# rsokolovskii/fl_scaling_sc_ldpc

Measured on AMD Instinct MI355X. Metric: MC codeword trials/sec, (4,8) SC-LDPC L=50 N=1000 eps=0.48 full BP, higher is better.
Workload: dtype u32

## Files before the change

### fl_scaling_sc_ldpc_amd/_lib.py

```python
import ctypes as C
import os

import numpy as np

HERE = os.path.dirname(os.path.abspath(__file__))
LIB_PATH = os.environ.get("SCLDPC_LIB_PATH") or os.path.join(HERE, "libscldpc_hip.so")

NCOUNTERS = 8
NRUN = 9
MAX_CAPS = 16
NPEELRUN = 8
PEELRUN_NAMES = ("trials", "fuckups", "lost", "fuckups_exp", "lost_exp", "blocks_exp")
COUNTER_NAMES = ("num_erasures", "num_blocks_err", "num_erasures_exp", "num_blocks_err_exp",
                 "num_erasures_p1", "iterations", "status", "channel_erasures")
RUN_NAMES = ("users_err", "frame_err", "frame_err_p1", "block_err", "users_err_exp", "frame_err_exp",
             "block_err_exp", "frames", "iterations")

EXPORTS = (
    "scldpc_abi_version", "scldpc_last_error", "scldpc_device_count",
    "scldpc_sample_glibc_host", "scldpc_glibc_state_bytes", "scldpc_glibc_state_init",
    "scldpc_glibc_state_reset_perm", "scldpc_sample_glibc_next_host",
    "scldpc_sample_philox_device", "scldpc_full_bp_device", "scldpc_sw_bp_device",
    "scldpc_accumulate_run_device", "scldpc_full_bp_lds_bytes",
    "scldpc_sample_philox_device_adj16", "scldpc_full_bp_device_adj16", "scldpc_sw_bp_device_adj16",
# ... 9 lines not shown
    "scldpc_sw_bp_ring_supported", "scldpc_cn_sockets_device", "scldpc_sw_bp_ring_device",
    "scldpc_accumulate_peel_device", "scldpc_clear_channel_range_device",
    "scldpc_stream_glibc_next_host", "scldpc_stream_run_device_inputs_at",
    "scldpc_full_bp_sock16_supported", "scldpc_full_bp_fixpoint_device_sock16", "scldpc_full_bp_device_sock16",
    "scldpc_full_bp_traj_device_cn16", "scldpc_full_bp_traj_device_sock16",
    "scldpc_full_bp_caps_device_cn16", "scldpc_full_bp_caps_device_sock16",
    "scldpc_full_bp_wide_supported", "scldpc_full_bp_device_wide", "scldpc_full_bp_traj_device_wide",
    "scldpc_full_bp_deg_supported", "scldpc_full_bp_deg_wide_supported", "scldpc_full_bp_fixpoint_device_deg",
    "scldpc_full_bp_device_deg", "scldpc_full_bp_traj_device_deg", "scldpc_full_bp_device_deg_wide",
    "scldpc_full_bp_traj_device_deg_wide",
    "scldpc_full_bp_caps_device_wide", "scldpc_full_bp_caps_device_deg", "scldpc_full_bp_caps_device_deg_wide",
    "scldpc_sw_bp_ring_deg_supported", "scldpc_sw_bp_ring_device_deg",
    "scldpc_stream_supported",
    "scldpc_swc_bp_ring_supported", "scldpc_swc_bp_ring_device",
    "scldpc_sample_philox_adj16_sock_supported", "scldpc_sample_philox_device_adj16_sock",
)


class ScldpcError(RuntimeError):
    pass


class CodeParams(C.Structure):
    _fields_ = [("dv", C.c_int32), ("dc", C.c_int32), ("L", C.c_int32), ("cns_pos", C.c_int32),
                ("vns_pos", C.c_int32)]

    @property
    def n(self):
        return self.vns_pos * self.L

    @property
    def nk(self):
        return (self.L + self.dv - 1) * self.cns_pos

    @property
    def nw(self):
        return (self.n + 31) // 32

    @property
    def edges(self):
        return self.n * self.dv

    def key(self):
        return (self.dv, self.dc, self.L, self.cns_pos, self.vns_pos)


_lib = None


def lib():
    global _lib
    if _lib is not None:
        return _lib
    if not os.path.exists(LIB_PATH):
        raise ScldpcError(f"{LIB_PATH} is missing — build it with `make -C fl_scaling_sc_ldpc_amd/csrc` "
                          "(hipcc, gfx950).  There is no CPU fallback.")
    import torch
    L = C.CDLL(LIB_PATH)
    P = C.POINTER
# ... 8 lines not shown
    L.scldpc_glibc_state_init.argtypes = [pp, u32, vp]
    L.scldpc_glibc_state_reset_perm.argtypes = [pp, vp]
    L.scldpc_sample_glibc_next_host.argtypes = [pp, vp, dbl, i32, vp, i32, vp, vp]
    L.scldpc_workspace_bytes.argtypes = [i32, pp, i32, i32, i32]
    L.scldpc_workspace_bytes.restype = i64
    L.scldpc_sample_philox_device.argtypes = [pp, u64, u64, i32, dbl, i32, vp, vp, vp, vp, u64, vp]
    L.scldpc_sample_philox_ensemble_device.argtypes = [pp, i32, u64, u64, i32, dbl, i32, vp, vp, vp, vp]
    L.scldpc_full_bp_fixpoint_device.argtypes = [pp, i32, vp, vp, i32, vp, vp, vp, u64, vp]
    L.scldpc_full_bp_fixpoint_device_adj16.argtypes = L.scldpc_full_bp_fixpoint_device.argtypes
    L.scldpc_sample_philox_cn16_supported.argtypes = [pp]
    L.scldpc_full_bp_cn16_supported.argtypes = [pp]
    L.scldpc_sample_philox_device_cn16.argtypes = [pp, u64, u64, i32, dbl, i32, vp, vp, vp, vp, vp]
    L.scldpc_sample_philox_sock16_supported.argtypes = [pp]
    L.scldpc_sample_philox_device_sock16.argtypes = [pp, u64, u64, i32, dbl, i32, vp, vp, vp, vp, vp]
    L.scldpc_sample_philox_adj16_sock_supported.argtypes = [pp]
    L.scldpc_sample_philox_device_adj16_sock.argtypes = [pp, u64, u64, i32, dbl, i32, vp, vp, vp, vp, vp, u64, vp]
    L.scldpc_full_bp_fixpoint_device_cn16.argtypes = [pp, i32, vp, vp, vp, i32, vp, vp, vp]
    L.scldpc_full_bp_device_cn16.argtypes = [pp, i32, vp, vp, vp, i32, i32, vp, vp, vp]
    L.scldpc_full_bp_sock16_supported.argtypes = [pp]
    L.scldpc_full_bp_fixpoint_device_sock16.argtypes = L.scldpc_full_bp_fixpoint_device_cn16.argtypes
    L.scldpc_full_bp_device_sock16.argtypes = L.scldpc_full_bp_device_cn16.argtypes
    L.scldpc_full_bp_traj_device_cn16.argtypes = [pp, i32, vp, vp, vp, i32, i32, vp, vp, i32, vp, vp]
    L.scldpc_full_bp_traj_device_sock16.argtypes = L.scldpc_full_bp_traj_device_cn16.argtypes
    L.scldpc_full_bp_caps_device_cn16.argtypes = [pp, i32, vp, vp, vp, i32, vp, i32, vp, vp]
    L.scldpc_full_bp_caps_device_sock16.argtypes = L.scldpc_full_bp_caps_device_cn16.argtypes
    L.scldpc_full_bp_wide_supported.argtypes = [pp]
    L.scldpc_full_bp_device_wide.argtypes = L.scldpc_full_bp_device_cn16.argtypes
    L.scldpc_full_bp_traj_device_wide.argtypes = L.scldpc_full_bp_traj_device_cn16.argtypes
    L.scldpc_full_bp_deg_supported.argtypes = [pp]
    L.scldpc_full_bp_deg_wide_supported.argtypes = [pp]
# ... 53 lines not shown
```

### fl_scaling_sc_ldpc_amd/csrc/sampler_v2.hip

```cpp
#include "common.h"
#include "kernel_util.h"
#include "philox.h"
#include <algorithm>
#include <cstdlib>

namespace {

using scldpc_dev::philox4x32_10;
using scldpc_dev::wave_inclusive_scan;

constexpr int kThreads = 1024;
constexpr int kWaves = kThreads / 64;
constexpr int kMaxDoped = 32;
constexpr int kWorkCap = 1024;

struct S2Args {
    int L, cns_pos, vns_pos, n, S, D, nb, nw;
    int ntrials;
    int force_exact;
    int ndoped;
    int doped[kMaxDoped];
    uint32_t seed_lo, seed_hi;
    unsigned long long trial0;
    uint32_t thresh;
    int off_gpk, off_fix, off_stage, off_wsum;
    uint16_t *vn_adj16;
    uint16_t *cn_adj16;
    uint32_t *chan;
};

template <int KMAX, int ROWS, int CNMODE, bool PERSIST = false>
__global__ __launch_bounds__(kThreads, KMAX == 1 ? 8 : 4) __attribute__((amdgpu_num_sgpr(72))) void sample_philox_v2_kernel(const S2Args a)
{
    constexpr int DV = 4, DC_SHIFT = 3, E = 4 * KMAX;
    constexpr int LG = ROWS == 1 ? 10 : ROWS == 2 ? 11 : ROWS == 4 ? 12 : 13;
    constexpr int KSHIFT = 32 - LG - 2;
    constexpr bool INCL = KMAX == 1;
    static_assert(ROWS * kThreads == (1 << LG) && (INCL ? ROWS <= 4 : ROWS == 8), "ROWS is 1, 2, 4 (KMAX 1) or 8 (KMAX 2)");
    extern __shared__ uint32_t lds[];
    uint32_t *hist = lds;
    uint32_t *gpk = lds + a.off_gpk;
    uint16_t *fix = reinterpret_cast<uint16_t *>(lds + a.off_fix);
    uint16_t *stage = reinterpret_cast<uint16_t *>(lds + a.off_stage);
    uint32_t *wsum = lds + a.off_wsum;
    uint32_t *wl = wsum + 32;

    const int tid = threadIdx.x, lane = tid & 63, wave = tid >> 6;
    const int S = a.S, nb = a.nb;
    const int ncalls = S >> 2;
    bool own[KMAX];
#pragma unroll
    for (int k = 0; k < KMAX; k++) own[k] = tid + k * kThreads < ncalls;
    auto sock = [&](int e) { return (uint32_t)((tid + (e >> 2) * kThreads) * 4 + (e & 3)); };
    auto stage_entry = [&](int p, uint32_t sck) -> uint16_t {
        const int u = (int)(sck & 3u), t = (int)(sck >> 2);
        if ((unsigned)(p - u) >= (unsigned)a.L) return (uint16_t)0xFFFFu;
        return CNMODE == 1 ? (uint16_t)((p - u) * a.vns_pos + t) : (uint16_t)sck;
    };

    auto nib_sum = [](uint32_t x) {
        const uint32_t v = (x & 0x0F0Fu) + ((x >> 4) & 0x0F0Fu);
        return (v + (v >> 8)) & 0xFFu;
    };
    auto load_words = [&](uint32_t (&x)[ROWS]) {
        if constexpr (ROWS % 4 == 0) {
#pragma unroll
            for (int r = 0; r < ROWS / 4; r++) {
                const uint4 q = reinterpret_cast<const uint4 *>(hist)[tid * (ROWS / 4) + r];
// ... 18 lines not shown
    const unsigned long long trial = a.trial0 + (unsigned long long)tr;
    const uint32_t t_lo = (uint32_t)trial, t_hi = (uint32_t)(trial >> 32);
    uint32_t rowP[KMAX], rowQ[KMAX], rowR[KMAX];
#pragma unroll
    for (int k = 0; k < KMAX; k++) rowP[k] = rowQ[k] = rowR[k] = 0;
    uint32_t nxt[E];
#pragma unroll
    for (int k = 0; k < KMAX; k++) {
        uint32_t r[4] = {0, 0, 0, 0};
        if (own[k]) philox4x32_10((uint32_t)(tid + k * kThreads), 0u, t_lo, t_hi, a.seed_lo, a.seed_hi, r);
#pragma unroll
        for (int u = 0; u < 4; u++) nxt[4 * k + u] = r[u];
    }
    for (int p = 0; p < a.D; p++) {
        STAMP(0);
        uint32_t key[E], slot[E], crowded = 0;
        auto word_of = [](uint32_t k) { return (k >> KSHIFT) & ~3u; };
        auto nib_of = [](uint32_t k) { return (k >> (KSHIFT - 2)) & 12u; };
#pragma unroll
        for (int e = 0; e < E; e++) {
            key[e] = nxt[e];
            const uint32_t sh = nib_of(key[e]);
            uint32_t *w = reinterpret_cast<uint32_t *>(reinterpret_cast<char *>(hist) + word_of(key[e]));
            slot[e] = (atomicAdd(w, (own[e >> 2] ? 1u : 0u) << sh) >> sh) & 0xFu;
            if constexpr (!INCL) crowded = max(crowded, slot[e]);
        }
        if (!INCL && crowded >= 15u) wsum[kWaves + 1] = 1u;
        __syncthreads();
        STAMP(1);

        bool ranked;
        if constexpr (INCL) {
            uint32_t x[ROWS], t20[ROWS], tot20 = 0;
            load_words(x);
#pragma unroll
            for (int r = 0; r < ROWS; r++) {
                x[r] *= 0x111110u;
                t20[r] = x[r] & 0xF00000u;
                tot20 += t20[r];
            }
            const uint32_t tot = tot20 >> 20, inc = wave_inclusive_scan(tot);
            if (lane == 63) wsum[wave] = inc;
            __syncthreads();
            uint32_t winc = lane < kWaves ? wsum[lane] : 0u;
            const uint32_t wt = winc;
            winc += (uint32_t)__builtin_amdgcn_update_dpp(0, (int)winc, 0x111, 0xF, 0xF, false);
            winc += (uint32_t)__builtin_amdgcn_update_dpp(0, (int)winc, 0x112, 0xF, 0xF, false);
            winc += (uint32_t)__builtin_amdgcn_update_dpp(0, (int)winc, 0x114, 0xF, 0xF, false);
            winc += (uint32_t)__builtin_amdgcn_update_dpp(0, (int)winc, 0x118, 0xF, 0xF, false);
            ranked = __builtin_amdgcn_readlane((int)winc, kWaves - 1) == S;
            uint32_t pre20 = (inc - tot + (uint32_t)__builtin_amdgcn_readlane((int)(winc - wt), wave)) << 20;
#pragma unroll
            for (int r = 0; r < ROWS; r++) {
                x[r] = (x[r] & 0xFFFF0u) | pre20;
                pre20 += t20[r];
            }
            store_words(x);
        } else {
            uint32_t x[ROWS], v[ROWS], tot = 0;
            load_words(x);
#pragma unroll
            for (int r = 0; r < ROWS; r++) v[r] = 0;
            if constexpr (ROWS % 2 == 0) {
#pragma unroll
                for (int r = 0; r < ROWS; r += 2) {
                    const uint32_t y = x[r] | (x[r + 1] << 16);
                    const uint32_t sb = (y & 0x0F0F0F0Fu) + ((y >> 4) & 0x0F0F0F0Fu);
                    v[r] = (sb & 0xFFu) + ((sb >> 8) & 0xFFu);
                    v[r + 1] = ((sb >> 16) & 0xFFu) + (sb >> 24);
                    tot += v[r] + v[r + 1];
// ... 6 lines not shown
            const uint32_t inc = wave_inclusive_scan(tot);
            if (lane == 63) wsum[wave] = inc;
            __syncthreads();
            const uint32_t wt = lane < kWaves ? wsum[lane] : 0u;
            const uint32_t winc = wave_inclusive_scan(wt);
            uint32_t pre = inc - tot + (uint32_t)__builtin_amdgcn_readlane((int)(winc - wt), wave);
#pragma unroll
            for (int r = 0; r < ROWS; r++) { x[r] |= pre << 16; pre += v[r]; }
            store_words(x);
        }
        __syncthreads();
        if constexpr (!INCL) ranked = wsum[kWaves + 1] == 0u;
        STAMP(2);

        if (ranked) {
            uint32_t rk[E], g0a[E], g1a[E];
            bool st[E];
            if constexpr (INCL) {
                uint32_t h[E];
#pragma unroll
                for (int e = 0; e < E; e++) h[e] = *reinterpret_cast<const uint32_t *>(reinterpret_cast<const char *>(hist) + word_of(key[e]));
#pragma unroll
                for (int e = 0; e < E; e++) {
                    const uint32_t t = h[e] >> nib_of(key[e]), pre = h[e] >> 20;
                    g0a[e] = pre + (t & 0xFu);
                    g1a[e] = pre + ((t >> 4) & 0xFu);
                    rk[e] = g0a[e] + slot[e];
                    st[e] = own[e >> 2] && ((g0a[e] ^ (g1a[e] - 1u)) >> DC_SHIFT) != 0u;
                }
            } else {
                uint32_t h[E];
#pragma unroll
                for (int e = 0; e < E; e++) h[e] = hist[own[e >> 2] ? (key[e] >> KSHIFT) >> 2 : 0u];
#pragma unroll
                for (int e = 0; e < E; e++) {
                    const uint32_t k4 = ((key[e] >> KSHIFT) & 3u) * 4u, x = h[e];
                    const uint32_t below = x & ((1u << k4) - 1u);
                    g0a[e] = (x >> 16) + (below & 0xFu) + ((below >> 4) & 0xFu) + ((below >> 8) & 0xFu);
                    g1a[e] = g0a[e] + ((x >> k4) & 0xFu);
                    rk[e] = g0a[e] + slot[e];
                    st[e] = own[e >> 2] && ((g1a[e] - 1u) >> DC_SHIFT) != (g0a[e] >> DC_SHIFT);
                }
            }
            if constexpr (INCL) {
                unsigned long long vote[E], anyv = 0;
                int total = 0;
#pragma unroll
                for (int e = 0; e < E; e++) { vote[e] = __builtin_amdgcn_ballot_w64(st[e]); anyv |= vote[e]; total += __builtin_popcountll(vote[e]); }
                if (anyv) {
                    int base = 0;
                    if (lane == 0) base = atomicAdd(reinterpret_cast<int *>(&wsum[kWaves]), total);
                    base = __builtin_amdgcn_readfirstlane(base);
                    const bool fits = base + total <= kWorkCap;
#pragma unroll
                    for (int e = 0; e < E; e++) {
                        if (st[e]) {
                            const uint32_t w = __builtin_amdgcn_mbcnt_hi((uint32_t)(vote[e] >> 32),
                                                                         __builtin_amdgcn_mbcnt_lo((uint32_t)vote[e], (uint32_t)base));
                            const uint32_t pk = (key[e] << LG) | sock(e);
                            gpk[rk[e]] = pk;
                            if (fits) { wl[2 * w] = g0a[e] | (g1a[e] << 16); wl[2 * w + 1] = pk; }
                        }
                        base += __builtin_popcountll(vote[e]);
                    }
                }
            } else {
                uint32_t smask = 0;
#pragma unroll
                for (int e = 0; e < E; e++) smask |= (st[e] ? 1u : 0u) << e;
                while (smask) {
                    const uint32_t e = (uint32_t)__ffs((int)smask) - 1u;
                    smask &= smask - 1u;
                    uint32_t ky = key[0], r0 = rk[0], g0 = g0a[0], g1 = g1a[0];
#pragma unroll
                    for (int f = 1; f < E; f++)
                        if (e == (uint32_t)f) { ky = key[f]; r0 = rk[f]; g0 = g0a[f]; g1 = g1a[f]; }
                    const uint32_t pk = (ky << LG) | (uint32_t)((tid + (int)(e >> 2) * kThreads) * 4 + (int)(e & 3u));
                    gpk[r0] = pk;
                    const int w = atomicAdd(reinterpret_cast<int *>(&wsum[kWaves]), 1);
                    if (w < kWorkCap) { wl[2 * w] = g0 | (g1 << 16); wl[2 * w + 1] = pk; }
                }
            }
#pragma unroll
            for (int k = 0; k < KMAX; k++) {
                if (!own[k]) continue;
                uint2 v;
                v.x = (rk[4 * k] >> DC_SHIFT) | ((rk[4 * k + 1] >> DC_SHIFT) << 16);
                v.y = (rk[4 * k + 2] >> DC_SHIFT) | ((rk[4 * k + 3] >> DC_SHIFT) << 16);
                reinterpret_cast<uint2 *>(fix)[tid + k * kThreads] = v;
            }
            if constexpr (CNMODE != 0) {
#pragma unroll
                for (int k = 0; k < KMAX; k++) {
                    if (!own[k]) continue;
#pragma unroll
                    for (int u = 0; u < 4; u++) stage[rk[4 * k + u]] = stage_entry(p, sock(4 * k + u));
                }
            }
        }
        __syncthreads();
        STAMP(3);

        {
            uint32_t z[ROWS];
#pragma unroll
            for (int r = 0; r < ROWS; r++) z[r] = 0;
            store_words(z);
            int nwork = (int)wsum[kWaves];
            const bool exact = !ranked || nwork > kWorkCap || a.force_exact == p || a.force_exact == -2;
            if (exact) {
                asm volatile("; ledger: cold");
                nwork = 0;
#pragma unroll
                for (int e = 0; e < E; e++) if (own[e >> 2]) gpk[sock(e)] = key[e];
                __syncthreads();
                uint32_t xr[E];
#pragma unroll
                for (int e = 0; e < E; e++) xr[e] = 0;
                for (int s2 = 0; s2 < S; s2++) {
                    const uint32_t k2 = gpk[s2];
#pragma unroll
                    for (int e = 0; e < E; e++) xr[e] += (k2 < key[e]) || (k2 == key[e] && (uint32_t)s2 < sock(e));
                }
#pragma unroll
                for (int k = 0; k < KMAX; k++) {
                    if (!own[k]) continue;
                    uint2 v;
                    v.x = (xr[4 * k] >> DC_SHIFT) | ((xr[4 * k + 1] >> DC_SHIFT) << 16);
                    v.y = (xr[4 * k + 2] >> DC_SHIFT) | ((xr[4 * k + 3] >> DC_SHIFT) << 16);
                    reinterpret_cast<uint2 *>(fix)[tid + k * kThreads] = v;
                    if constexpr (CNMODE != 0) {
#pragma unroll
                        for (int u = 0; u < 4; u++) stage[xr[4 * k + u]] = stage_entry(p, sock(4 * k + u));
                    }
                }
            }
            for (int w = tid; w < nwork; w += kThreads) {
                const uint32_t ea = wl[2 * w], pk = wl[2 * w + 1];
                uint32_t r = ea & 0xFFFFu;
#pragma unroll 1
                for (uint32_t m = ea & 0xFFFFu; m < (ea >> 16); m++) r += gpk[m] < pk;
                const uint32_t sck = pk & ((1u << LG) - 1u);
                if constexpr (CNMODE != 0) stage[r] = stage_entry(p, sck);
                fix[sck] = (uint16_t)(r >> DC_SHIFT);
            }
        }
        if (p + 1 < a.D) {
            uint32_t k_lo = a.seed_lo, k_hi = a.seed_hi;
            asm volatile("" : "+s"(k_lo), "+s"(k_hi));
#pragma unroll
            for (int k = 0; k < KMAX; k++) {
                uint32_t r[4] = {0, 0, 0, 0};
                if (own[k]) philox4x32_10((uint32_t)(tid + k * kThreads), (uint32_t)(p + 1), t_lo, t_hi, k_lo, k_hi, r);
#pragma unroll
                for (int u = 0; u < 4; u++) nxt[4 * k + u] = r[u];
            }
        }
        __syncthreads();
        if (tid == 0) { wsum[kWaves] = 0; wsum[kWaves + 1] = 0; }
        STAMP(4);

        const int qpos = p - (DV - 1);
#pragma unroll
        for (int k = 0; k < KMAX; k++) {
            uint2 c = make_uint2(0u, 0u);
            if (own[k]) c = reinterpret_cast<const uint2 *>(fix)[tid + k * kThreads];
            if (qpos >= 0 && own[k]) {
                const size_t j = (size_t)tr * a.n + (size_t)qpos * a.vns_pos + (size_t)(tid + k * kThreads);
// ... 31 lines not shown
            if (lo < hi) word &= ~(((hi - lo) == 32 ? 0xFFFFFFFFu : ((1u << (hi - lo)) - 1u)) << lo);
        }
        chan[w] = word;
    }
    STAMP(6);
    };
    if constexpr (PERSIST) {
        for (int tr = blockIdx.x; tr < a.ntrials; tr += gridDim.x) {
            sample_trial(tr);
            __syncthreads();
        }
    } else {
        sample_trial((int)blockIdx.x);
    }
    STAMP_FLUSH();
}


__device__ __forceinline__ uint32_t wl_entry_vn(const S2Args &a, int p, uint32_t sck)
{
    return (uint32_t)((p - (int)(sck & 3u)) * a.vns_pos + (int)(sck >> 2));
}

template <int LG, int CNMODE>
__global__ __launch_bounds__(kThreads, 8) __attribute__((amdgpu_num_sgpr(72))) void sample_philox_v3_kernel(const S2Args a)
{
    constexpr int DV = 4, DC_SHIFT = 3, E = 4;
    constexpr int NB = 1 << LG, ROWS = NB / kThreads;
    constexpr int KSHIFT = 32 - LG - 2;
    constexpr uint32_t LOWMASK = (1u << KSHIFT) - 1u;
// ... 234 lines not shown
#pragma unroll
            for (int u = 0; u < 4; u++) word |= (uint32_t)((r[u] >> 1) < a.thresh) << (c * 4 + u);
        }
        const int j0 = w * 32;
        if (j0 + 32 > a.n) word &= (1u << (a.n - j0)) - 1u;
        for (int d = 0; d < a.ndoped; d++) {
            const int lo = max(a.doped[d] * a.vns_pos, j0) - j0, hi = min((a.doped[d] + 1) * a.vns_pos, j0 + 32) - j0;
            if (lo < hi) word &= ~(((hi - lo) == 32 ? 0xFFFFFFFFu : ((1u << (hi - lo)) - 1u)) << lo);
        }
        chan[w] = word;
    }
    STAMP(8);
    STAMP_FLUSH();
}

int launch_v2(const char *who, int cnmode, const scldpc_code_params *p, uint64_t seed, uint64_t trial0, int32_t ntrials,
              double eps, int32_t ndoped, const int32_t *doped_positions, uint16_t *d_vn_adj16, uint16_t *d_table,
              uint32_t *d_chan_bits, void *stream)
{
    if (ntrials < 0 || (ntrials > 0 && (!d_vn_adj16 || !d_chan_bits)))
        return scldpc::set_error(SCLDPC_ERR_BAD_ARG, "%s: null buffer or negative ntrials", who);
    if (ndoped < 0 || ndoped > kMaxDoped || (ndoped > 0 && !doped_positions))
        return scldpc::set_error(SCLDPC_ERR_BAD_ARG, "%s: 0 <= ndoped <= %d", who, kMaxDoped);
    if (!(eps >= 0.0 && eps <= 1.0))
        return scldpc::set_error(SCLDPC_ERR_BAD_ARG, "%s: eps=%g outside [0,1]", who, eps);
    if (ntrials == 0) return SCLDPC_OK;
    if (!d_table) cnmode = 0;

    S2Args a{};
    a.L = p->L; a.cns_pos = p->cns_pos; a.vns_pos = p->vns_pos;
    a.n = scldpc::n_of(p); a.S = p->cns_pos * p->dc; a.D = p->L + p->dv - 1; a.nw = scldpc::nw_of(p);
    int lg = 10;
    while ((1 << lg) < a.S) lg++;
    a.nb = 1 << lg;
    a.ndoped = ndoped;
    for (int d = 0; d < ndoped; d++) {
        if (doped_positions[d] < 0 || doped_positions[d] >= p->L)
            return scldpc::set_error(SCLDPC_ERR_BAD_ARG, "doped position %d outside [0,%d)", doped_positions[d], p->L);
        a.doped[d] = doped_positions[d];
    }
    a.seed_lo = (uint32_t)seed; a.seed_hi = (uint32_t)(seed >> 32);
    a.trial0 = trial0;
    {
        const double x = eps * 2147483647.0;
        double c = (double)(uint64_t)x;
        if (c < x) c += 1.0;
        a.thresh = (uint32_t)c;
    }
    const char *gen_env = getenv("SCLDPC_SAMPLER_GEN");
    const bool v3 = a.nb <= 4 * kThreads && gen_env && atoi(gen_env) == 3;
    int off = ((v3 ? 2 : 1) * a.nb + 3) & ~3;
    a.off_gpk = off;   off += (a.S + 3) & ~3;
    a.off_fix = off;   off += (a.S / 2 + 3) & ~3;
    a.off_stage = off; off += cnmode ? (a.S / 2 + 3) & ~3 : 0;
    a.off_wsum = off;  off += 32 + 2 * kWorkCap;
    size_t lds_bytes = 4u * (size_t)off;
    lds_bytes = std::min(lds_bytes + scldpc::debug_lds_pad("SAMPLER"), std::max(lds_bytes, (size_t)scldpc::kMaxLdsBytes));
    if (lds_bytes > (size_t)scldpc::kMaxLdsBytes)
        return scldpc::set_error(SCLDPC_ERR_TOO_LARGE, "%s: %zu bytes of LDS per trial", who, lds_bytes);
    a.vn_adj16 = d_vn_adj16; a.cn_adj16 = d_table; a.chan = d_chan_bits;
    a.ntrials = ntrials;
    a.force_exact = -1;
    if (const char *v = getenv("SCLDPC_DEBUG_SAMPLER_EXACT_POS")) a.force_exact = atoi(v);

    using Kern = void (*)(const S2Args);
    static const Kern table[4][3] = {
        {sample_philox_v2_kernel<1, 1, 0>, sample_philox_v2_kernel<1, 1, 1>, sample_philox_v2_kernel<1, 1, 2>},
        {sample_philox_v2_kernel<1, 2, 0>, sample_philox_v2_kernel<1, 2, 1>, sample_philox_v2_kernel<1, 2, 2>},
        {sample_philox_v2_kernel<1, 4, 0>, sample_philox_v2_kernel<1, 4, 1>, sample_philox_v2_kernel<1, 4, 2>},
        {sample_philox_v2_kernel<2, 8, 0>, sample_philox_v2_kernel<2, 8, 1>, sample_philox_v2_kernel<2, 8, 2>},
    };
    const int rows = a.nb / kThreads;
    static const Kern table3[3][3] = {
        {sample_philox_v3_kernel<10, 0>, sample_philox_v3_kernel<10, 1>, sample_philox_v3_kernel<10, 2>},
        {sample_philox_v3_kernel<11, 0>, sample_philox_v3_kernel<11, 1>, sample_philox_v3_kernel<11, 2>},
        {sample_philox_v3_kernel<12, 0>, sample_philox_v3_kernel<12, 1>, sample_philox_v3_kernel<12, 2>},
    };
    const int grid = v3 ? ntrials : scldpc::debug_grid("SAMPLER", ntrials);
    Kern kern = v3 ? table3[lg - 10][cnmode] : table[rows == 1 ? 0 : rows == 2 ? 1 : rows == 4 ? 2 : 3][cnmode];
    if (grid < ntrials && rows == 4 && cnmode == 1) kern = sample_philox_v2_kernel<1, 4, 1, true>;
    else if (grid < ntrials) return scldpc::set_error(SCLDPC_ERR_BAD_ARG, "SCLDPC_DEBUG_GRID_SAMPLER: only the <1,4,1> kernel has a persistent form");
    if (int rc_ = scldpc::allow_max_lds(reinterpret_cast<const void *>(kern))) return rc_;
    hipLaunchKernelGGL(kern, dim3(grid), dim3(kThreads), lds_bytes, static_cast<hipStream_t>(stream), a);
    SCLDPC_HIP_CHECK(hipGetLastError());
    return SCLDPC_OK;
}

bool v2_shape(const scldpc_code_params *p)
{
    if (scldpc::check_params(p)) return false;
    const int S = p->cns_pos * p->dc;
    return p->dv == 4 && p->dc == 8 && (S & 3) == 0 && S <= 8192 && p->vns_pos * p->dv == S;
}

}

extern "C" int scldpc_sample_philox_cn16_supported(const scldpc_code_params *p)
{
    return v2_shape(p) && scldpc::n_of(p) < 65535;
}

extern "C" int scldpc_sample_philox_sock16_supported(const scldpc_code_params *p)
{
    return v2_shape(p);
}

extern "C" int scldpc_sample_philox_device_cn16(const scldpc_code_params *p, uint64_t seed, uint64_t trial0,
                                                int32_t ntrials, double eps, int32_t ndoped,
                                                const int32_t *doped_positions, uint16_t *d_vn_adj16,
// ... 26 lines not shown
```

### fl_scaling_sc_ldpc_amd/engine.py

```python
import ctypes as C
import os

import numpy as np
import torch

from . import _lib
from ._lib import (CodeParams, MAX_CAPS, NCOUNTERS, NRUN, NPEELRUN, COUNTER_NAMES, RUN_NAMES, PEELRUN_NAMES, ScldpcError,
                   check, lib)


def make_params(dv=4, dc=8, L=50, N=1000):
    if (N * dv) % dc:
        raise ValueError(f"N*dv must be divisible by dc (N={N}, dv={dv}, dc={dc})")
    return CodeParams(dv, dc, L, N * dv // dc, N)


def _stream_ptr(device):
    return C.c_void_p(torch.cuda.current_stream(device).cuda_stream)


WS_SAMPLE, WS_FULL_BP, WS_SW_BP, WS_PEEL_SWEEP, WS_PEEL_PICK = range(5)


def _workspace(op, p, ntrials, device, arg0=0, arg1=0):
# ... 137 lines not shown

def sw_ring_supported(p, W):
    return bool(lib().scldpc_sw_bp_ring_supported(C.byref(p), int(W)))


def sw_ring_deg_supported(p, W):
    return bool(lib().scldpc_sw_bp_ring_deg_supported(C.byref(p), int(W)))


def swc_ring_supported(p, W):
    return bool(lib().scldpc_swc_bp_ring_supported(C.byref(p), int(W)))


def sock16_supported(p):
    return bool(lib().scldpc_sample_philox_sock16_supported(C.byref(p)))


def sample_philox_sock16(p, seed, trial0, ntrials, eps, doped=(), device="cuda:0", out=None):
    return _sample_philox_tables(lib().scldpc_sample_philox_device_sock16, p, seed, trial0, ntrials, eps, doped, device, out)


def sample_philox_sock_supported(p):
    return bool(lib().scldpc_sample_philox_adj16_sock_supported(C.byref(p)))


def sample_philox_sock(p, seed, trial0, ntrials, eps, doped=(), device="cuda:0", out=None):
    _require_gpu()
    if out is None:
        d_adj = torch.empty((ntrials, p.n, p.dv), dtype=torch.int16, device=device)
        d_cn = torch.empty((ntrials, p.nk, p.dc), dtype=torch.int16, device=device)
# ... 426 lines not shown
```

### include/scldpc.h

```cpp
#ifndef SCLDPC_H
#define SCLDPC_H
#include <stdint.h>

#ifdef __cplusplus
extern "C" {
#endif

#define SCLDPC_ABI_VERSION 2

enum {
    SCLDPC_OK = 0,
    SCLDPC_ERR_BAD_ARG = -1,
    SCLDPC_ERR_TOO_LARGE = -2,
    SCLDPC_ERR_HIP = -3,
    SCLDPC_ERR_NO_DEVICE = -4
};

enum { SCLDPC_WS_SAMPLE = 0, SCLDPC_WS_FULL_BP = 1, SCLDPC_WS_SW_BP = 2, SCLDPC_WS_PEEL_SWEEP = 3, SCLDPC_WS_PEEL_PICK = 4 };
struct scldpc_code_params;
int64_t scldpc_workspace_bytes(int32_t op, const struct scldpc_code_params *p, int32_t ntrials, int32_t arg0, int32_t arg1);

typedef struct scldpc_code_params {
    int32_t dv;
    int32_t dc;
// ... 57 lines not shown
int scldpc_full_bp_fixpoint_device(const scldpc_code_params *p, int32_t ntrials,
                                   const int32_t *d_vn_adj, const uint32_t *d_chan_bits, int32_t is_term,
                                   int32_t *d_counters, uint32_t *d_erased_bits, void *d_workspace, uint64_t workspace_bytes, void *stream);
int scldpc_full_bp_fixpoint_device_adj16(const scldpc_code_params *p, int32_t ntrials,
                                         const uint16_t *d_vn_adj16, const uint32_t *d_chan_bits, int32_t is_term,
                                         int32_t *d_counters, uint32_t *d_erased_bits, void *d_workspace, uint64_t workspace_bytes, void *stream);

int scldpc_sample_philox_cn16_supported(const scldpc_code_params *p);
int scldpc_sample_philox_sock16_supported(const scldpc_code_params *p);
int scldpc_sample_philox_device_sock16(const scldpc_code_params *p, uint64_t seed, uint64_t trial0, int32_t ntrials,
                                       double eps, int32_t ndoped, const int32_t *doped_positions, uint16_t *d_vn_adj16,
                                       uint16_t *d_cn_sock16, uint32_t *d_chan_bits, void *stream);
int scldpc_sample_philox_device_cn16(const scldpc_code_params *p, uint64_t seed, uint64_t trial0, int32_t ntrials,
                                     double eps, int32_t ndoped, const int32_t *doped_positions, uint16_t *d_vn_adj16,
                                     uint16_t *d_cn_adj16, uint32_t *d_chan_bits, void *stream);
int scldpc_sample_philox_adj16_sock_supported(const scldpc_code_params *p);
int scldpc_sample_philox_device_adj16_sock(const scldpc_code_params *p, uint64_t seed, uint64_t trial0, int32_t ntrials,
                                           double eps, int32_t ndoped, const int32_t *doped_positions, uint16_t *d_vn_adj16,
                                           uint16_t *d_cn_sock16, uint32_t *d_chan_bits, void *d_workspace,
                                           uint64_t workspace_bytes, void *stream);
int scldpc_full_bp_cn16_supported(const scldpc_code_params *p);
int scldpc_full_bp_fixpoint_device_cn16(const scldpc_code_params *p, int32_t ntrials, const uint16_t *d_vn_adj16,
                                        const uint16_t *d_cn_adj16, const uint32_t *d_chan_bits, int32_t is_term,
                                        int32_t *d_counters, uint32_t *d_erased_bits, void *stream);
int scldpc_full_bp_device_cn16(const scldpc_code_params *p, int32_t ntrials, const uint16_t *d_vn_adj16,
                               const uint16_t *d_cn_adj16, const uint32_t *d_chan_bits, int32_t max_it, int32_t is_term,
                               int32_t *d_counters, uint32_t *d_erased_bits, void *stream);
int scldpc_full_bp_sock16_supported(const scldpc_code_params *p);
int scldpc_full_bp_fixpoint_device_sock16(const scldpc_code_params *p, int32_t ntrials, const uint16_t *d_vn_adj16,
                                          const uint16_t *d_cn_sock16, const uint32_t *d_chan_bits, int32_t is_term,
// ... 161 lines not shown
```

Before: 1.215 million.

## Add opt-in 512-thread sampler workgroup and restructure ranking per call

Adds a 512-thread variant of the v2 Philox sampler kernel for 2048 < S <= 4096, selected only through SCLDPC_SAMPLER_WG=512, with a smaller work list and an occupancy check. It also restructures the ranked path to process each 4-socket call separately, packs slot nibbles into one register, and drops the kept t20 array for large ROWS, all to lower register pressure. Shape computation moves into a shared helper that is exported for Python. With the default setting the 1024-thread kernel still runs, but it also picks up the register-saving restructuring.

```diff
diff --git a/fl_scaling_sc_ldpc_amd/_lib.py b/fl_scaling_sc_ldpc_amd/_lib.py
--- a/fl_scaling_sc_ldpc_amd/_lib.py
+++ b/fl_scaling_sc_ldpc_amd/_lib.py
@@ -47,6 +47,7 @@
     "scldpc_stream_supported",
     "scldpc_swc_bp_ring_supported", "scldpc_swc_bp_ring_device",
     "scldpc_sample_philox_adj16_sock_supported", "scldpc_sample_philox_device_adj16_sock",
+    "scldpc_sampler_v2_shape",
 )
 
 
@@ -76,6 +77,11 @@
 
     def key(self):
         return (self.dv, self.dc, self.L, self.cns_pos, self.vns_pos)
+
+
+class SamplerShape(C.Structure):
+    _fields_ = [(k, C.c_int32) for k in ("gen", "threads", "kmax", "rows", "cnmode", "nb", "work_cap", "off_gpk", "off_fix",
+                                         "off_stage", "off_wsum", "lds_bytes")]
 
 
 _lib = None
@@ -114,6 +120,7 @@
     L.scldpc_sample_philox_sock16_supported.argtypes = [pp]
     L.scldpc_sample_philox_device_sock16.argtypes = [pp, u64, u64, i32, dbl, i32, vp, vp, vp, vp, vp]
     L.scldpc_sample_philox_adj16_sock_supported.argtypes = [pp]
+    L.scldpc_sampler_v2_shape.argtypes = [i32, i32, i32, i32, P(SamplerShape)]
     L.scldpc_sample_philox_device_adj16_sock.argtypes = [pp, u64, u64, i32, dbl, i32, vp, vp, vp, vp, vp, u64, vp]
     L.scldpc_full_bp_fixpoint_device_cn16.argtypes = [pp, i32, vp, vp, vp, i32, vp, vp, vp]
     L.scldpc_full_bp_device_cn16.argtypes = [pp, i32, vp, vp, vp, i32, i32, vp, vp, vp]
diff --git a/fl_scaling_sc_ldpc_amd/csrc/sampler_v2.hip b/fl_scaling_sc_ldpc_amd/csrc/sampler_v2.hip
--- a/fl_scaling_sc_ldpc_amd/csrc/sampler_v2.hip
+++ b/fl_scaling_sc_ldpc_amd/csrc/sampler_v2.hip
@@ -2,6 +2,7 @@
 #include "kernel_util.h"
 #include "philox.h"
 #include <algorithm>
+#include <atomic>
 #include <cstdlib>
 
 namespace {
@@ -13,6 +14,7 @@
 constexpr int kWaves = kThreads / 64;
 constexpr int kMaxDoped = 32;
 constexpr int kWorkCap = 1024;
+constexpr int kWorkCap512 = 512;
 
 struct S2Args {
     int L, cns_pos, vns_pos, n, S, D, nb, nw;
@@ -27,16 +29,21 @@
     uint16_t *vn_adj16;
     uint16_t *cn_adj16;
     uint32_t *chan;
+    int work_cap;
 };
 
-template <int KMAX, int ROWS, int CNMODE, bool PERSIST = false>
-__global__ __launch_bounds__(kThreads, KMAX == 1 ? 8 : 4) __attribute__((amdgpu_num_sgpr(72))) void sample_philox_v2_kernel(const S2Args a)
-{
-    constexpr int DV = 4, DC_SHIFT = 3, E = 4 * KMAX;
-    constexpr int LG = ROWS == 1 ? 10 : ROWS == 2 ? 11 : ROWS == 4 ? 12 : 13;
+template <int THREADS, int KMAX, int ROWS, int CNMODE, bool PERSIST>
+__device__ __forceinline__ void sample_philox_v2(const S2Args &a)
+{
+    constexpr int kThreads = THREADS, kWaves = THREADS / 64;
+    constexpr int kWorkCap = THREADS == 512 ? kWorkCap512 : 1024;
+    constexpr int DV = 4, DC_SHIFT = 3, E = 4 * KMAX, NB = ROWS * THREADS;
+    constexpr int LG = NB == 1024 ? 10 : NB == 2048 ? 11 : NB == 4096 ? 12 : 13;
     constexpr int KSHIFT = 32 - LG - 2;
-    constexpr bool INCL = KMAX == 1;
-    static_assert(ROWS * kThreads == (1 << LG) && (INCL ? ROWS <= 4 : ROWS == 8), "ROWS is 1, 2, 4 (KMAX 1) or 8 (KMAX 2)");
+    constexpr bool INCL = NB <= 4096;
+    static_assert(NB == (1 << LG) && NB <= 4 * KMAX * THREADS && (THREADS == 1024 || (THREADS == 512 && KMAX == 2 && !PERSIST)),
+                  "nb = 1024 .. 8192 words, a socket slot for every word, 1024 threads or 512 with two calls each");
+    const int work_cap = THREADS == 512 ? a.work_cap : kWorkCap;
     extern __shared__ uint32_t lds[];
     uint32_t *hist = lds;
     uint32_t *gpk = lds + a.off_gpk;
@@ -51,7 +58,8 @@
     bool own[KMAX];
 #pragma unroll
     for (int k = 0; k < KMAX; k++) own[k] = tid + k * kThreads < ncalls;
-    auto sock = [&](int e) { return (uint32_t)((tid + (e >> 2) * kThreads) * 4 + (e & 3)); };
+    auto tid_here = [&]() { int t = tid; if constexpr (THREADS == 512) asm volatile("" : "+v"(t)); return t; };
+    auto sock_of = [&](int t, int e) { return (uint32_t)((t + (e >> 2) * kThreads) * 4 + (e & 3)); };
     auto stage_entry = [&](int p, uint32_t sck) -> uint16_t {
         const int u = (int)(sck & 3u), t = (int)(sck >> 2);
         if ((unsigned)(p - u) >= (unsigned)a.L) return (uint16_t)0xFFFFu;
@@ -100,7 +108,10 @@
     }
     for (int p = 0; p < a.D; p++) {
         STAMP(0);
-        uint32_t key[E], slot[E], crowded = 0;
+        constexpr bool PACKED = INCL && KMAX == 2;
+        uint32_t key[E], slot[PACKED ? 1 : E], crowded = 0;
+        if constexpr (PACKED) slot[0] = 0;
+        auto slot_of = [&](int e) { if constexpr (PACKED) return (slot[0] >> (4 * (E - 1 - e))) & 0xFu; else return slot[e]; };
         auto word_of = [](uint32_t k) { return (k >> KSHIFT) & ~3u; };
         auto nib_of = [](uint32_t k) { return (k >> (KSHIFT - 2)) & 12u; };
 #pragma unroll
@@ -108,8 +119,9 @@
             key[e] = nxt[e];
             const uint32_t sh = nib_of(key[e]);
             uint32_t *w = reinterpret_cast<uint32_t *>(reinterpret_cast<char *>(hist) + word_of(key[e]));
-            slot[e] = (atomicAdd(w, (own[e >> 2] ? 1u : 0u) << sh) >> sh) & 0xFu;
-            if constexpr (!INCL) crowded = max(crowded, slot[e]);
+            const uint32_t sl = (atomicAdd(w, (own[e >> 2] ? 1u : 0u) << sh) >> sh) & 0xFu;
+            if constexpr (PACKED) slot[0] = (slot[0] << 4) | sl; else slot[e] = sl;
+            if constexpr (!INCL) crowded = max(crowded, sl);
         }
         if (!INCL && crowded >= 15u) wsum[kWaves + 1] = 1u;
         __syncthreads();
@@ -117,13 +129,15 @@
 
         bool ranked;
         if constexpr (INCL) {
-            uint32_t x[ROWS], t20[ROWS], tot20 = 0;
+            constexpr bool KEEP = ROWS <= 4;
+            uint32_t x[ROWS], t20[KEEP ? ROWS : 1], tot20 = 0;
             load_words(x);
 #pragma unroll
             for (int r = 0; r < ROWS; r++) {
                 x[r] *= 0x111110u;
-                t20[r] = x[r] & 0xF00000u;
-                tot20 += t20[r];
+                const uint32_t t = x[r] & 0xF00000u;
+                if constexpr (KEEP) t20[r] = t;
+                tot20 += t;
             }
             const uint32_t tot = tot20 >> 20, inc = wave_inclusive_scan(tot);
             if (lane == 63) wsum[wave] = inc;
@@ -133,13 +147,14 @@
             winc += (uint32_t)__builtin_amdgcn_update_dpp(0, (int)winc, 0x111, 0xF, 0xF, false);
             winc += (uint32_t)__builtin_amdgcn_update_dpp(0, (int)winc, 0x112, 0xF, 0xF, false);
             winc += (uint32_t)__builtin_amdgcn_update_dpp(0, (int)winc, 0x114, 0xF, 0xF, false);
-            winc += (uint32_t)__builtin_amdgcn_update_dpp(0, (int)winc, 0x118, 0xF, 0xF, false);
+            if constexpr (kWaves > 8) winc += (uint32_t)__builtin_amdgcn_update_dpp(0, (int)winc, 0x118, 0xF, 0xF, false);
             ranked = __builtin_amdgcn_readlane((int)winc, kWaves - 1) == S;
             uint32_t pre20 = (inc - tot + (uint32_t)__builtin_amdgcn_readlane((int)(winc - wt), wave)) << 20;
 #pragma unroll
             for (int r = 0; r < ROWS; r++) {
+                const uint32_t t = KEEP ? t20[r] : x[r] & 0xF00000u;
                 x[r] = (x[r] & 0xFFFF0u) | pre20;
-                pre20 += t20[r];
+                pre20 += t;
             }
             store_words(x);
         } else {
@@ -176,22 +191,61 @@
         STAMP(2);
 
         if (ranked) {
-            uint32_t rk[E], g0a[E], g1a[E];
-            bool st[E];
+            auto store_call = [&](int k, const uint32_t *rk4) {
+                if (!own[k]) return;
+                const int tq = tid_here();
+                uint2 v;
+                v.x = (rk4[0] >> DC_SHIFT) | ((rk4[1] >> DC_SHIFT) << 16);
+                v.y = (rk4[2] >> DC_SHIFT) | ((rk4[3] >> DC_SHIFT) << 16);
+                reinterpret_cast<uint2 *>(fix)[tid + k * kThreads] = v;
+                if constexpr (CNMODE != 0) {
+#pragma unroll
+                    for (int u = 0; u < 4; u++) stage[rk4[u]] = stage_entry(p, sock_of(tq, 4 * k + u));
+                }
+            };
             if constexpr (INCL) {
                 uint32_t h[E];
 #pragma unroll
                 for (int e = 0; e < E; e++) h[e] = *reinterpret_cast<const uint32_t *>(reinterpret_cast<const char *>(hist) + word_of(key[e]));
 #pragma unroll
-                for (int e = 0; e < E; e++) {
-                    const uint32_t t = h[e] >> nib_of(key[e]), pre = h[e] >> 20;
-                    g0a[e] = pre + (t & 0xFu);
-                    g1a[e] = pre + ((t >> 4) & 0xFu);
-                    rk[e] = g0a[e] + slot[e];
-                    st[e] = own[e >> 2] && ((g0a[e] ^ (g1a[e] - 1u)) >> DC_SHIFT) != 0u;
+                for (int k = 0; k < KMAX; k++) {
+                    uint32_t rk[4], g0a[4], g1a[4];
+                    bool st[4];
+#pragma unroll
+                    for (int u = 0; u < 4; u++) {
+                        const int e = 4 * k + u;
+                        const uint32_t t = h[e] >> nib_of(key[e]), pre = h[e] >> 20;
+                        g0a[u] = pre + (t & 0xFu);
+                        g1a[u] = pre + ((t >> 4) & 0xFu);
+                        rk[u] = g0a[u] + slot_of(e);
+                        st[u] = own[k] && ((g0a[u] ^ (g1a[u] - 1u)) >> DC_SHIFT) != 0u;
+                    }
+                    unsigned long long vote[4], anyv = 0;
+                    int total = 0;
+#pragma unroll
+                    for (int u = 0; u < 4; u++) { vote[u] = __builtin_amdgcn_ballot_w64(st[u]); anyv |= vote[u]; total += __builtin_popcountll(vote[u]); }
+                    if (anyv) {
+                        int base = 0;
+                        if (lane == 0) base = atomicAdd(reinterpret_cast<int *>(&wsum[kWaves]), total);
+                        base = __builtin_amdgcn_readfirstlane(base);
+                        const bool fits = base + total <= work_cap;
+#pragma unroll
+                        for (int u = 0; u < 4; u++) {
+                            if (st[u]) {
+                                const uint32_t w = __builtin_amdgcn_mbcnt_hi((uint32_t)(vote[u] >> 32),
+                                                                             __builtin_amdgcn_mbcnt_lo((uint32_t)vote[u], (uint32_t)base));
+                                const uint32_t pk = (key[4 * k + u] << LG) | sock_of(tid_here(), 4 * k + u);
+                                gpk[rk[u]] = pk;
+                                if (fits) { wl[2 * w] = g0a[u] | (g1a[u] << 16); wl[2 * w + 1] = pk; }
+                            }
+                            base += __builtin_popcountll(vote[u]);
+                        }
+                    }
+                    store_call(k, rk);
                 }
             } else {
-                uint32_t h[E];
+                uint32_t rk[E], g0a[E], g1a[E], h[E];
+                bool st[E];
 #pragma unroll
                 for (int e = 0; e < E; e++) h[e] = hist[own[e >> 2] ? (key[e] >> KSHIFT) >> 2 : 0u];
 #pragma unroll
@@ -200,33 +254,9 @@
                     const uint32_t below = x & ((1u << k4) - 1u);
                     g0a[e] = (x >> 16) + (below & 0xFu) + ((below >> 4) & 0xFu) + ((below >> 8) & 0xFu);
                     g1a[e] = g0a[e] + ((x >> k4) & 0xFu);
-                    rk[e] = g0a[e] + slot[e];
+                    rk[e] = g0a[e] + slot_of(e);
                     st[e] = own[e >> 2] && ((g1a[e] - 1u) >> DC_SHIFT) != (g0a[e] >> DC_SHIFT);
                 }
-            }
-            if constexpr (INCL) {
-                unsigned long long vote[E], anyv = 0;
-                int total = 0;
-#pragma unroll
-                for (int e = 0; e < E; e++) { vote[e] = __builtin_amdgcn_ballot_w64(st[e]); anyv |= vote[e]; total += __builtin_popcountll(vote[e]); }
-                if (anyv) {
-                    int base = 0;
-                    if (lane == 0) base = atomicAdd(reinterpret_cast<int *>(&wsum[kWaves]), total);
-                    base = __builtin_amdgcn_readfirstlane(base);
-                    const bool fits = base + total <= kWorkCap;
-#pragma unroll
-                    for (int e = 0; e < E; e++) {
-                        if (st[e]) {
-                            const uint32_t w = __builtin_amdgcn_mbcnt_hi((uint32_t)(vote[e] >> 32),
-                                                                         __builtin_amdgcn_mbcnt_lo((uint32_t)vote[e], (uint32_t)base));
-                            const uint32_t pk = (key[e] << LG) | sock(e);
-                            gpk[rk[e]] = pk;
-                            if (fits) { wl[2 * w] = g0a[e] | (g1a[e] << 16); wl[2 * w + 1] = pk; }
-                        }
-                        base += __builtin_popcountll(vote[e]);
-                    }
-                }
-            } else {
                 uint32_t smask = 0;
 #pragma unroll
                 for (int e = 0; e < E; e++) smask |= (st[e] ? 1u : 0u) << e;
@@ -240,24 +270,10 @@
                     const uint32_t pk = (ky << LG) | (uint32_t)((tid + (int)(e >> 2) * kThreads) * 4 + (int)(e & 3u));
                     gpk[r0] = pk;
                     const int w = atomicAdd(reinterpret_cast<int *>(&wsum[kWaves]), 1);
-                    if (w < kWorkCap) { wl[2 * w] = g0 | (g1 << 16); wl[2 * w + 1] = pk; }
-                }
-            }
-#pragma unroll
-            for (int k = 0; k < KMAX; k++) {
-                if (!own[k]) continue;
-                uint2 v;
-                v.x = (rk[4 * k] >> DC_SHIFT) | ((rk[4 * k + 1] >> DC_SHIFT) << 16);
-                v.y = (rk[4 * k + 2] >> DC_SHIFT) | ((rk[4 * k + 3] >> DC_SHIFT) << 16);
-                reinterpret_cast<uint2 *>(fix)[tid + k * kThreads] = v;
-            }
-            if constexpr (CNMODE != 0) {
-#pragma unroll
-                for (int k = 0; k < KMAX; k++) {
-                    if (!own[k]) continue;
-#pragma unroll
-                    for (int u = 0; u < 4; u++) stage[rk[4 * k + u]] = stage_entry(p, sock(4 * k + u));
-                }
+                    if (w < work_cap) { wl[2 * w] = g0 | (g1 << 16); wl[2 * w + 1] = pk; }
+                }
+#pragma unroll
+                for (int k = 0; k < KMAX; k++) store_call(k, rk + 4 * k);
             }
         }
         __syncthreads();
@@ -269,12 +285,13 @@
             for (int r = 0; r < ROWS; r++) z[r] = 0;
             store_words(z);
             int nwork = (int)wsum[kWaves];
-            const bool exact = !ranked || nwork > kWorkCap || a.force_exact == p || a.force_exact == -2;
+            const bool exact = !ranked || nwork > work_cap || a.force_exact == p || a.force_exact == -2;
             if (exact) {
                 asm volatile("; ledger: cold");
                 nwork = 0;
-#pragma unroll
-                for (int e = 0; e < E; e++) if (own[e >> 2]) gpk[sock(e)] = key[e];
+                const int tq = tid_here();
+#pragma unroll
+                for (int e = 0; e < E; e++) if (own[e >> 2]) gpk[sock_of(tq, e)] = key[e];
                 __syncthreads();
                 uint32_t xr[E];
 #pragma unroll
@@ -282,7 +299,7 @@
                 for (int s2 = 0; s2 < S; s2++) {
                     const uint32_t k2 = gpk[s2];
 #pragma unroll
-                    for (int e = 0; e < E; e++) xr[e] += (k2 < key[e]) || (k2 == key[e] && (uint32_t)s2 < sock(e));
+                    for (int e = 0; e < E; e++) xr[e] += (k2 < key[e]) || (k2 == key[e] && (uint32_t)s2 < sock_of(tq, e));
                 }
 #pragma unroll
                 for (int k = 0; k < KMAX; k++) {
@@ -293,7 +310,7 @@
                     reinterpret_cast<uint2 *>(fix)[tid + k * kThreads] = v;
                     if constexpr (CNMODE != 0) {
 #pragma unroll
-                        for (int u = 0; u < 4; u++) stage[xr[4 * k + u]] = stage_entry(p, sock(4 * k + u));
+                        for (int u = 0; u < 4; u++) stage[xr[4 * k + u]] = stage_entry(p, sock_of(tq, 4 * k + u));
                     }
                 }
             }
@@ -313,7 +330,7 @@
 #pragma unroll
             for (int k = 0; k < KMAX; k++) {
                 uint32_t r[4] = {0, 0, 0, 0};
-                if (own[k]) philox4x32_10((uint32_t)(tid + k * kThreads), (uint32_t)(p + 1), t_lo, t_hi, k_lo, k_hi, r);
+                if (own[k]) philox4x32_10((uint32_t)(tid_here() + k * kThreads), (uint32_t)(p + 1), t_lo, t_hi, k_lo, k_hi, r);
 #pragma unroll
                 for (int u = 0; u < 4; u++) nxt[4 * k + u] = r[u];
             }
@@ -375,6 +392,18 @@
         sample_trial((int)blockIdx.x);
     }
     STAMP_FLUSH();
+}
+
+template <int KMAX, int ROWS, int CNMODE, bool PERSIST = false>
+__global__ __launch_bounds__(kThreads, KMAX == 1 ? 8 : 4) __attribute__((amdgpu_num_sgpr(72))) void sample_philox_v2_kernel(const S2Args a)
+{
+    sample_philox_v2<kThreads, KMAX, ROWS, CNMODE, PERSIST>(a);
+}
+
+template <int CNMODE>
+__global__ __launch_bounds__(512, 6) void sample_philox_v2_wg512_kernel(const S2Args a)
+{
+    sample_philox_v2<512, 2, 8, CNMODE, false>(a);
 }
 
 
@@ -639,6 +668,40 @@
     STAMP_FLUSH();
 }
 
+constexpr bool kWg512ByDefault = false;
+
+int v2_shape_of(const char *who, int S, int cnmode, int wg, int gen, scldpc_sampler_shape *sh)
+{
+    if (S < 4 || S > 8192 || (S & 3) || cnmode < 0 || cnmode > 2)
+        return scldpc::set_error(SCLDPC_ERR_BAD_ARG, "%s: sockets per position S=%d (a multiple of 4, at most 8192), cnmode=%d", who, S, cnmode);
+    if (wg != 0 && wg != 512 && wg != 1024)
+        return scldpc::set_error(SCLDPC_ERR_BAD_ARG, "%s: SCLDPC_SAMPLER_WG is 1024 or 512 (got %d)", who, wg);
+    int lg = 10;
+    while ((1 << lg) < S) lg++;
+    const int nb = 1 << lg;
+    const bool v3 = nb <= 4 * kThreads && gen == 3;
+    const bool fits512 = S > 2048 && S <= 4096;
+    if (wg == 512 && !fits512)
+        return scldpc::set_error(SCLDPC_ERR_BAD_ARG, "%s: SCLDPC_SAMPLER_WG=512 takes 2048 < S <= 4096 sockets per position (got %d)", who, S);
+    if (wg == 512 && v3)
+        return scldpc::set_error(SCLDPC_ERR_BAD_ARG, "%s: SCLDPC_SAMPLER_WG=512 with SCLDPC_SAMPLER_GEN=3: the third generation has 1024 threads", who);
+    const bool w512 = !v3 && fits512 && (wg == 512 || (wg == 0 && kWg512ByDefault));
+    sh->gen = v3 ? 3 : 2;
+    sh->threads = w512 ? 512 : kThreads;
+    sh->kmax = v3 ? 1 : (S + 4 * sh->threads - 1) / (4 * sh->threads);
+    sh->rows = nb / sh->threads;
+    sh->cnmode = cnmode;
+    sh->nb = nb;
+    sh->work_cap = w512 ? kWorkCap512 : kWorkCap;
+    int off = ((v3 ? 2 : 1) * nb + 3) & ~3;
+    sh->off_gpk = off;   off += (S + 3) & ~3;
+    sh->off_fix = off;   off += (S / 2 + 3) & ~3;
+    sh->off_stage = off; off += cnmode ? (S / 2 + 3) & ~3 : 0;
+    sh->off_wsum = off;  off += 32 + 2 * sh->work_cap;
+    sh->lds_bytes = 4 * off;
+    return SCLDPC_OK;
+}
+
 int launch_v2(const char *who, int cnmode, const scldpc_code_params *p, uint64_t seed, uint64_t trial0, int32_t ntrials,
               double eps, int32_t ndoped, const int32_t *doped_positions, uint16_t *d_vn_adj16, uint16_t *d_table,
               uint32_t *d_chan_bits, void *stream)
@@ -655,9 +718,6 @@
     S2Args a{};
     a.L = p->L; a.cns_pos = p->cns_pos; a.vns_pos = p->vns_pos;
     a.n = scldpc::n_of(p); a.S = p->cns_pos * p->dc; a.D = p->L + p->dv - 1; a.nw = scldpc::nw_of(p);
-    int lg = 10;
-    while ((1 << lg) < a.S) lg++;
-    a.nb = 1 << lg;
     a.ndoped = ndoped;
     for (int d = 0; d < ndoped; d++) {
         if (doped_positions[d] < 0 || doped_positions[d] >= p->L)
@@ -672,15 +732,19 @@
         if (c < x) c += 1.0;
         a.thresh = (uint32_t)c;
     }
-    const char *gen_env = getenv("SCLDPC_SAMPLER_GEN");
-    const bool v3 = a.nb <= 4 * kThreads && gen_env && atoi(gen_env) == 3;
-    int off = ((v3 ? 2 : 1) * a.nb + 3) & ~3;
-    a.off_gpk = off;   off += (a.S + 3) & ~3;
-    a.off_fix = off;   off += (a.S / 2 + 3) & ~3;
-    a.off_stage = off; off += cnmode ? (a.S / 2 + 3) & ~3 : 0;
-    a.off_wsum = off;  off += 32 + 2 * kWorkCap;
-    size_t lds_bytes = 4u * (size_t)off;
-    lds_bytes = std::min(lds_bytes + scldpc::debug_lds_pad("SAMPLER"), std::max(lds_bytes, (size_t)scldpc::kMaxLdsBytes));
+    const char *gen_env = getenv("SCLDPC_SAMPLER_GEN"), *wg_env = getenv("SCLDPC_SAMPLER_WG");
+    scldpc_sampler_shape sh{};
+    if (int rc_ = v2_shape_of(who, a.S, cnmode, wg_env ? atoi(wg_env) : 0, gen_env ? atoi(gen_env) : 0, &sh)) return rc_;
+    const bool v3 = sh.gen == 3, w512 = sh.threads == 512;
+    const int lg = __builtin_ctz((unsigned)sh.nb);
+    a.nb = sh.nb;
+    a.off_gpk = sh.off_gpk; a.off_fix = sh.off_fix; a.off_stage = sh.off_stage; a.off_wsum = sh.off_wsum;
+    a.work_cap = sh.work_cap;
+    if (const char *v = getenv("SCLDPC_DEBUG_SAMPLER_WORKCAP"))
+        a.work_cap = std::min(sh.work_cap, std::max(0, atoi(v)));
+    const size_t pad = scldpc::debug_lds_pad("SAMPLER");
+    size_t lds_bytes = (size_t)sh.lds_bytes;
+    lds_bytes = std::min(lds_bytes + pad, std::max(lds_bytes, (size_t)scldpc::kMaxLdsBytes));
     if (lds_bytes > (size_t)scldpc::kMaxLdsBytes)
         return scldpc::set_error(SCLDPC_ERR_TOO_LARGE, "%s: %zu bytes of LDS per trial", who, lds_bytes);
     a.vn_adj16 = d_vn_adj16; a.cn_adj16 = d_table; a.chan = d_chan_bits;
@@ -695,6 +759,7 @@
         {sample_philox_v2_kernel<1, 4, 0>, sample_philox_v2_kernel<1, 4, 1>, sample_philox_v2_kernel<1, 4, 2>},
         {sample_philox_v2_kernel<2, 8, 0>, sample_philox_v2_kernel<2, 8, 1>, sample_philox_v2_kernel<2, 8, 2>},
     };
+    static const Kern table512[3] = {sample_philox_v2_wg512_kernel<0>, sample_philox_v2_wg512_kernel<1>, sample_philox_v2_wg512_kernel<2>};
     const int rows = a.nb / kThreads;
     static const Kern table3[3][3] = {
         {sample_philox_v3_kernel<10, 0>, sample_philox_v3_kernel<10, 1>, sample_philox_v3_kernel<10, 2>},
@@ -702,11 +767,22 @@
         {sample_philox_v3_kernel<12, 0>, sample_philox_v3_kernel<12, 1>, sample_philox_v3_kernel<12, 2>},
     };
     const int grid = v3 ? ntrials : scldpc::debug_grid("SAMPLER", ntrials);
-    Kern kern = v3 ? table3[lg - 10][cnmode] : table[rows == 1 ? 0 : rows == 2 ? 1 : rows == 4 ? 2 : 3][cnmode];
+    Kern kern = v3 ? table3[lg - 10][cnmode] : w512 ? table512[cnmode] : table[rows == 1 ? 0 : rows == 2 ? 1 : rows == 4 ? 2 : 3][cnmode];
+    if (grid < ntrials && w512) return scldpc::set_error(SCLDPC_ERR_BAD_ARG, "SCLDPC_DEBUG_GRID_SAMPLER: the 512-thread form has no persistent launch");
     if (grid < ntrials && rows == 4 && cnmode == 1) kern = sample_philox_v2_kernel<1, 4, 1, true>;
     else if (grid < ntrials) return scldpc::set_error(SCLDPC_ERR_BAD_ARG, "SCLDPC_DEBUG_GRID_SAMPLER: only the <1,4,1> kernel has a persistent form");
     if (int rc_ = scldpc::allow_max_lds(reinterpret_cast<const void *>(kern))) return rc_;
-    hipLaunchKernelGGL(kern, dim3(grid), dim3(kThreads), lds_bytes, static_cast<hipStream_t>(stream), a);
+    if (w512 && pad == 0) {
+        static std::atomic<bool> resident[3];
+        if (!resident[cnmode].load(std::memory_order_acquire)) {
+            int nblk = 0;
+            SCLDPC_HIP_CHECK(hipOccupancyMaxActiveBlocksPerMultiprocessor(&nblk, reinterpret_cast<const void *>(kern), sh.threads, lds_bytes));
+            if (nblk < 3)
+                return scldpc::set_error(SCLDPC_ERR_HIP, "%s: %d workgroups of 512 threads and %zu bytes of LDS per CU, not three", who, nblk, lds_bytes);
+            resident[cnmode].store(true, std::memory_order_release);
+        }
+    }
+    hipLaunchKernelGGL(kern, dim3(grid), dim3(sh.threads), lds_bytes, static_cast<hipStream_t>(stream), a);
     SCLDPC_HIP_CHECK(hipGetLastError());
     return SCLDPC_OK;
 }
@@ -718,6 +794,12 @@
     return p->dv == 4 && p->dc == 8 && (S & 3) == 0 && S <= 8192 && p->vns_pos * p->dv == S;
 }
 
+}
+
+extern "C" int scldpc_sampler_v2_shape(int32_t sockets_per_pos, int32_t cnmode, int32_t wg, int32_t gen, scldpc_sampler_shape *shape)
+{
+    if (!shape) return scldpc::set_error(SCLDPC_ERR_BAD_ARG, "scldpc_sampler_v2_shape: null shape");
+    return v2_shape_of("scldpc_sampler_v2_shape", sockets_per_pos, cnmode, wg, gen, shape);
 }
 
 extern "C" int scldpc_sample_philox_cn16_supported(const scldpc_code_params *p)
diff --git a/fl_scaling_sc_ldpc_amd/engine.py b/fl_scaling_sc_ldpc_amd/engine.py
--- a/fl_scaling_sc_ldpc_amd/engine.py
+++ b/fl_scaling_sc_ldpc_amd/engine.py
@@ -175,6 +175,12 @@
 
 def sock16_supported(p):
     return bool(lib().scldpc_sample_philox_sock16_supported(C.byref(p)))
+
+
+def sampler_v2_shape(S, cnmode, wg=0, gen=0):
+    sh = _lib.SamplerShape()
+    check(lib().scldpc_sampler_v2_shape(int(S), int(cnmode), int(wg), int(gen), C.byref(sh)))
+    return sh
 
 
 def sample_philox_sock16(p, seed, trial0, ntrials, eps, doped=(), device="cuda:0", out=None):
diff --git a/include/scldpc.h b/include/scldpc.h
--- a/include/scldpc.h
+++ b/include/scldpc.h
@@ -95,6 +95,13 @@
 int scldpc_sample_philox_device_cn16(const scldpc_code_params *p, uint64_t seed, uint64_t trial0, int32_t ntrials,
                                      double eps, int32_t ndoped, const int32_t *doped_positions, uint16_t *d_vn_adj16,
                                      uint16_t *d_cn_adj16, uint32_t *d_chan_bits, void *stream);
+typedef struct scldpc_sampler_shape {
+    int32_t gen, threads, kmax, rows, cnmode;
+    int32_t nb, work_cap;
+    int32_t off_gpk, off_fix, off_stage, off_wsum;
+    int32_t lds_bytes;
+} scldpc_sampler_shape;
+int scldpc_sampler_v2_shape(int32_t sockets_per_pos, int32_t cnmode, int32_t wg, int32_t gen, scldpc_sampler_shape *shape);
 int scldpc_sample_philox_adj16_sock_supported(const scldpc_code_params *p);
 int scldpc_sample_philox_device_adj16_sock(const scldpc_code_params *p, uint64_t seed, uint64_t trial0, int32_t ntrials,
                                            double eps, int32_t ndoped, const int32_t *doped_positions, uint16_t *d_vn_adj16,
```

Result: no change. 1.215 million, median of 4 (+0.0%).
